# NVlabs/L4P

Hardware: AMD Instinct MI355X
Metric: frames/sec (all heads), 16x224x224 clip; encoder MFMA-roofline % (higher is better)
Workload: dtype bf16; 1 GPU; configs[2]: single MI355X, all heads (depth+flow+track2d/3d+motion-seg+pose), bf16, batch=4 clips, 64 track queries per clip; parallelism=dp1 (clips sharded, no collective in the step)

## Files before the change

### include/l4p_hip.h

```cpp
#ifndef L4P_HIP_H
#define L4P_HIP_H

#include <stddef.h>
#include <stdint.h>

#ifdef __cplusplus
extern "C" {
#endif

#define L4P_BF16 0
#define L4P_F32 1
#define L4P_F16 2

#define L4P_OK 0
#define L4P_E_INVALID (-1)
#define L4P_E_HIP (-2)
#define L4P_E_MISSING (-3)

typedef void* l4p_stream;
typedef struct l4p_engine l4p_engine;

const char* l4p_last_error(void);
int l4p_abi_version(void);

// ... 36 lines not shown
    float* out_f32;
    void* out_T;
    long long ldc;
    int epi;
    void* vt;
    int S, H, Dp;
    int kt, kh, kw, Cout;
    int a_gr, a_gs, a_go;
    int c_gr, c_gs, c_go;
    void* out_relu_T;
    void* k_tiled;
    int splitk;
    float* partial;
    const float* hyper;
    int hyper_rows;
    float q_scale;
    int tuning;
    int w_gr;
    long long w_gs;
    int b_gs;
    long long o_gs;
    int ups_hi, ups_wi;
    int kw_cols, kw_len;
} l4p_gemm_desc;

int l4p_gemm(l4p_stream stream, int dtype, const l4p_gemm_desc* d);
#define L4P_GEMM_GROUP_MAX 4
int l4p_gemm_group(l4p_stream stream, int dtype, const l4p_gemm_desc* d, int n);
int l4p_conv3d_k3(l4p_stream stream, int dtype, const l4p_gemm_desc* d);
int l4p_conv3d_subpixel(l4p_stream stream, int dtype, const l4p_gemm_desc* d);

int l4p_layernorm(l4p_stream stream, int dtype, const float* x, const float* gamma, const float* beta, float eps,
                  void* out_T, float* out_f32, int M, int C);

#define L4P_ATTN_PRESCALED 0.0f
int l4p_attention(l4p_stream stream, int dtype, const void* q, const void* kt, const void* vt, void* out, int B, int S,
                  int H, int Dh, float scale);

int l4p_patch_gather(l4p_stream stream, int dtype, const float* rgb, void* out, int B, int Cin, int T, int H, int W,
                     int pt, int ph, int pw, int Kp);

int l4p_cast(l4p_stream stream, int dtype, const float* x, void* y, long long n);

int l4p_upsample_trilinear(l4p_stream stream, int dtype, const void* x, void* y, int B, int Ti, int Hi, int Wi, int To,
                           int Ho, int Wo, int C, int align_corners);

// ... 225 lines not shown
```

### l4p_amd/_lib.py

```python
from __future__ import annotations

import ctypes as C
import os
from typing import Optional

L4P_BF16 = 0
L4P_F32 = 1
L4P_F16 = 2

ABI_VERSION = 17

EPI_DENSE, EPI_QKV, EPI_CONVT, EPI_MASKDOT = 0, 1, 2, 3
ACT_NONE, ACT_GELU, ACT_RELU = 0, 1, 2

_HERE = os.path.dirname(os.path.abspath(__file__))
LIB_PATH = os.environ.get("L4P_HIP_LIB") or os.path.join(_HERE, "lib", "libl4p_hip.so")


class GemmDesc(C.Structure):

    _fields_ = [
        ("A", C.c_void_p), ("lda", C.c_longlong),
        ("W", C.c_void_p), ("ldw", C.c_longlong),
        ("M", C.c_int), ("N", C.c_int), ("K", C.c_int),
        ("Ti", C.c_int), ("Hi", C.c_int), ("Wi", C.c_int), ("Cin", C.c_int),
        ("To", C.c_int), ("Ho", C.c_int), ("Wo", C.c_int),
        ("st", C.c_int), ("sh", C.c_int), ("sw", C.c_int), ("relu_in", C.c_int),
        ("bias", C.c_void_p), ("act", C.c_int),
        ("res1", C.c_void_p), ("res2", C.c_void_p), ("res_f32", C.c_int),
        ("ldr", C.c_longlong), ("res_mod", C.c_int),
        ("out_f32", C.c_void_p), ("out_T", C.c_void_p), ("ldc", C.c_longlong),
        ("epi", C.c_int),
        ("vt", C.c_void_p), ("S", C.c_int), ("H", C.c_int), ("Dp", C.c_int),
        ("kt", C.c_int), ("kh", C.c_int), ("kw", C.c_int), ("Cout", C.c_int),
        ("a_gr", C.c_int), ("a_gs", C.c_int), ("a_go", C.c_int),
        ("c_gr", C.c_int), ("c_gs", C.c_int), ("c_go", C.c_int),
        ("out_relu_T", C.c_void_p),
        ("k_tiled", C.c_void_p),
        ("splitk", C.c_int), ("partial", C.c_void_p),
        ("hyper", C.c_void_p), ("hyper_rows", C.c_int),
        ("q_scale", C.c_float), ("tuning", C.c_int),
        ("w_gr", C.c_int), ("w_gs", C.c_longlong), ("b_gs", C.c_int), ("o_gs", C.c_longlong),
        ("ups_hi", C.c_int), ("ups_wi", C.c_int),
        ("kw_cols", C.c_int), ("kw_len", C.c_int),
    ]


class EncoderCfg(C.Structure):

    _fields_ = [
        ("dim", C.c_int), ("depth", C.c_int), ("heads", C.c_int), ("head_dim", C.c_int), ("mlp_hidden", C.c_int),
        ("in_chans", C.c_int), ("frames", C.c_int), ("img_h", C.c_int), ("img_w", C.c_int),
        ("pt", C.c_int), ("ph", C.c_int), ("pw", C.c_int),
        ("patch_kp", C.c_int), ("ln_eps", C.c_float),
    ]


class DptCfg(C.Structure):

    _fields_ = [
        ("dim", C.c_int), ("nt", C.c_int), ("nh", C.c_int), ("nw", C.c_int),
        ("layer_dims", C.c_int * 4),
        ("feature_dim", C.c_int), ("last_dim", C.c_int), ("out_ch", C.c_int),
        ("actpost", (C.c_int * 3) * 4), ("fusion", (C.c_int * 3) * 4),
        ("out_t", C.c_int), ("out_h", C.c_int), ("out_w", C.c_int),
        ("post_exp", C.c_int),
    ]
# ... 166 lines not shown
```

### l4p_amd/csrc/api.hip

```cpp
#include <stdarg.h>
#include <stdio.h>
#include <string.h>

#include <string>
#include <unordered_map>
#include <vector>

#include <stdlib.h>

#include "engine.hpp"

static thread_local char g_err[512] = "";

void l4p_set_error(const char* fmt, ...) {
    va_list ap;
    va_start(ap, fmt);
    vsnprintf(g_err, sizeof(g_err), fmt, ap);
    va_end(ap);
}

int launch_layernorm_res(int dtype, const float* x, int x_mod, const void* delta_T, const float* gamma, const float* beta, float eps,
                         void* out_T, float* out_f32, int M, int C, const float* add, int add_mod, void* out_T2, const float* x_shared,
                         int x_period, int x_split, hipStream_t stream, float* out_sum = nullptr, const float* part = nullptr,
                         int nsplit = 0, const float* pbias = nullptr, float* out_stats = nullptr);

extern "C" {

const char* l4p_last_error(void) { return g_err; }
int l4p_abi_version(void) { return 17; }

int l4p_stream_create_cu_mask(int first_cu, int n_cus, l4p_stream* out) {
    if (!out || first_cu < 0 || n_cus < 1 || first_cu + n_cus > 1024) {
        l4p_set_error("l4p_stream_create_cu_mask: bad CU range [%d, %d)", first_cu, first_cu + n_cus);
        return L4P_E_INVALID;
    }
    uint32_t mask[32] = {0};
    for (int c = first_cu; c < first_cu + n_cus; ++c) mask[c >> 5] |= 1u << (c & 31);
    hipStream_t s = nullptr;
    HIP_TRY(hipExtStreamCreateWithCUMask(&s, (uint32_t)((first_cu + n_cus + 31) / 32), mask));
    *out = (l4p_stream)s;
    return 0;
}
int l4p_stream_destroy(l4p_stream s) {
    HIP_TRY(hipStreamDestroy((hipStream_t)s));
    return 0;
}

int l4p_gemm(l4p_stream stream, int dtype, const l4p_gemm_desc* d) {
    if (!d) {
        l4p_set_error("l4p_gemm: null descriptor");
        return L4P_E_INVALID;
    }
// ... 396 lines not shown
```

### l4p_amd/csrc/api_dpt.hip

```cpp
#include <string.h>

#include <string>

#include "engine.hpp"

namespace {

struct Bump {
    char* base;
    size_t off, cap;
    bool dry;
    void* take(size_t bytes) {
        const size_t a = (off + 255) & ~(size_t)255;
        off = a + bytes;
        return dry ? (void*)1 : (off <= cap ? base + a : nullptr);
    }
};

struct Vol {
    void* p;
    int t, h, w, c;
    long long vox(int B) const { return (long long)B * t * h * w; }
};

// ... 97 lines not shown
        if (rc || dry) return o;
        GemmParams p;
        memset(&p, 0, sizeof(p));
        p.A = x.p;
        p.W = W(wk);
        p.ldw = (long long)(k[0] == 1 ? 3 : 2) * (k[1] == 1 ? 3 : 2) * (k[2] == 1 ? 3 : 2) * x.c;
        p.M = (int)x.vox(B);
        p.N = k[0] * k[1] * k[2] * cout;
        p.K = (int)p.ldw;
        p.Ti = x.t;
        p.Hi = x.h;
        p.Wi = x.w;
        p.Cin = x.c;
        p.bias = (const float*)W(bk);
        p.out_T = o.p;
        p.out_relu_T = relu_copy ? relu_copy->p : nullptr;
        p.kt = k[0];
        p.kh = k[1];
        p.kw = k[2];
        p.Cout = cout;
        if (!rc) rc = launch_gemm(dt, 2, p, st);
        return o;
    }
    Vol conv3(const Vol& x_in, const char* wk, const char* bk, int cout, const int s[3], int act, const void* r1, const void* r2,
              Vol* relu_copy, int ups_h = 0, int ups_w = 0) {
        Vol x = x_in;
        if (ups_h > 0) x.h = ups_h, x.w = ups_w;
        Vol o = vol((x.t - 1) / s[0] + 1, (x.h - 1) / s[1] + 1, (x.w - 1) / s[2] + 1, cout);
        if (relu_copy) *relu_copy = vol(o.t, o.h, o.w, cout);
        const long long M = o.vox(B);
        const int sk = ups_h > 0 ? 1 : splitk_for(M, cout, 27 * x.c, es);
        float* partial = sk > 1 ? (float*)alloc((size_t)sk * M * cout * 4) : nullptr;
        if (rc || dry) return o;
        GemmParams p;
        memset(&p, 0, sizeof(p));
        p.A = x.p;
        p.W = W(wk);
        p.ldw = 27 * x.c;
        p.M = (int)M;
        p.N = cout;
        p.K = 27 * x.c;
        p.Ti = x.t;
        p.Hi = x.h;
        p.Wi = x.w;
        p.Cin = x.c;
        p.To = o.t;
        p.Ho = o.h;
        p.Wo = o.w;
        p.st = s[0];
        p.sh = s[1];
        p.sw = s[2];
        p.bias = bk ? (const float*)W(bk) : nullptr;
        p.act = act;
        if (r1) {
            p.res1 = r1;
            p.res2 = r2;
            p.res_f32 = 0;
            p.ldr = cout;
        }
        p.out_T = o.p;
        p.ldc = cout;
        p.out_relu_T = relu_copy ? relu_copy->p : nullptr;
        p.splitk = sk;
        p.partial = partial;
        if (ups_h > 0) p.ups_hi = x_in.h, p.ups_wi = x_in.w;
        if (!rc) rc = launch_gemm(dt, 1, p, st);
        return o;
    }
    Vol resize(const Vol& x, int t, int h, int w) {
        if (t == x.t && h == x.h && w == x.w) return x;
        Vol o = vol(t, h, w, x.c);
        if (rc || dry) return o;
        rc = launch_upsample(dt, x.p, o.p, B, x.t, x.h, x.w, t, h, w, x.c, 1, st);
        return o;
    }
};

int run(Ctx& c, const l4p_dpt_cfg* cfg, const void* const* hooks, float* out) {
    static const int one[3] = {1, 1, 1};
    const int F = cfg->feature_dim;
    Vol lay[4], layr[4];
    for (int i = 0; i < 4; ++i) {
        Vol tok{(void*)hooks[i], cfg->nt, cfg->nh, cfg->nw, cfg->dim};
        char wk[32], bk[32];
        snprintf(wk, sizeof(wk), "act%d.0.w", i);
        snprintf(bk, sizeof(bk), "act%d.0.b", i);
        Vol a = c.dense(tok, wk, bk, cfg->layer_dims[i]);
        const int* sf = cfg->actpost[i];
// ... 39 lines not shown
                return L4P_E_INVALID;
            }
            o = rcu(r, 1, lay[i], layr[i], p4.p, &orl);
        }
        Vol o2 = rcu(r, 2, o, orl, nullptr, nullptr);
        char wk[32], bk[32];
        snprintf(wk, sizeof(wk), "ref%d.out.w", r);
        snprintf(bk, sizeof(bk), "ref%d.out.b", r);
        Vol oc = c.dense(o2, wk, bk, F);
        const int* fs = cfg->fusion[i];
        path = c.resize(oc, oc.t * fs[0], oc.h * fs[1], oc.w * fs[2]);
        if (c.rc) return c.rc;
    }
    Vol h1 = c.conv3(path, "head1.w", "head1.b", F / 2, one, ACT_NONE, nullptr, nullptr, nullptr);
    Vol h2;
    const bool fuse = is16(c.dt) && knob(KNOB_CONV_UPS) && cfg->out_t == h1.t && (cfg->out_h != h1.h || cfg->out_w != h1.w) &&
                      cfg->last_dim == 128 && h1.c % 32 == 0 && cfg->out_t % 2 == 0 && cfg->out_h % 16 == 0 && cfg->out_w % 16 == 0 &&
                      (long long)c.B * cfg->out_t * cfg->out_h * cfg->out_w / 512 >= 192 &&
                      (long long)c.B * cfg->out_t * cfg->out_h * cfg->out_w * h1.c * 2 < (1ll << 32);
    if (fuse && !c.dry) {
        h2 = c.conv3(h1, "head2.w", "head2.b", cfg->last_dim, one, ACT_RELU, nullptr, nullptr, nullptr, cfg->out_h, cfg->out_w);
    } else {
        Vol h1u = c.resize(h1, cfg->out_t, cfg->out_h, cfg->out_w);
        h2 = c.conv3(h1u, "head2.w", "head2.b", cfg->last_dim, one, ACT_RELU, nullptr, nullptr, nullptr);
    }
    if (c.rc || c.dry) return c.rc;
    return launch_head_out(c.dt, h2.p, (const float*)c.W("out.w"), (const float*)c.W("out.b"), out,
                           (long long)h2.t * h2.h * h2.w, c.B, cfg->last_dim, cfg->out_ch, cfg->post_exp, c.st);
}

}

extern "C" {

size_t l4p_dpt_workspace_bytes(const l4p_engine* e, const l4p_dpt_cfg* cfg, int B) {
    if (!e || !cfg || B <= 0) return 0;
    Ctx c;
    c.e = e;
    c.st = nullptr;
    c.dt = e->dtype;
    c.es = esize_of(e->dtype);
    c.B = B;
    c.ws = Bump{nullptr, 0, 0, true};
    c.dry = true;
    const void* hooks[4] = {(void*)1, (void*)1, (void*)1, (void*)1};
    run(c, cfg, hooks, nullptr);
// ... 21 lines not shown
```

### l4p_amd/csrc/conv3_halo.hpp

```cpp
#pragma once
#include "gemm.hpp"

template <int WR, int WC>
struct ConvHaloCfg {
    static constexpr int BM = WR * 128, BN = WC * 64, CK = 32;
    static constexpr int TT = 2, TW = 16, TH = BM / (TT * TW);
    static constexpr int HH = TH + 2, HW = TW + 2, PR = HH * HW, NPL = TT + 2;
    static constexpr int PRP = (PR + 15) / 16 * 16;
    static constexpr int HALO_BYTES = NPL * PRP * 64;
    static constexpr int WSLOT = BN * 64, NSLOT = 4;
    static constexpr int LDS_BYTES = HALO_BYTES + NSLOT * WSLOT;
    static constexpr int W_PASS = BN * 4 / 512;
    static constexpr int H_PASS = (PRP * 4 + 511) / 512;
};

template <typename T, int WR, int WC, bool UPS = false>
__global__ __launch_bounds__(512) void conv3_halo_kernel(const GemmParams p) {
    static_assert(WR * WC == 8 && (WC == 2 || WC == 4), "8 waves");
    typedef ConvHaloCfg<WR, WC> Cfg;
    constexpr int BM = Cfg::BM, BN = Cfg::BN, TM = 8, TN = 4;
    constexpr int TT = Cfg::TT, TH = Cfg::TH, TW = Cfg::TW, HH = Cfg::HH, HW = Cfg::HW, PR = Cfg::PR, PRP = Cfg::PRP;
    constexpr int WSLOT = Cfg::WSLOT, W_PASS = Cfg::W_PASS, H_PASS = Cfg::H_PASS;
    static_assert(2 * H_PASS <= 9, "planes 2 / 3 are refilled before tap 9");
    typedef const __attribute__((address_space(1))) void* gptr_t;
    typedef __attribute__((address_space(3))) void* lptr_t;

    extern __shared__ __attribute__((aligned(16))) char smem[];
    char* const wring = smem + Cfg::HALO_BYTES;

    const int tid = threadIdx.x, lane = tid & 63;
    const int wave = __builtin_amdgcn_readfirstlane(tid >> 6);
    const int wr = wave / WC, wc = wave % WC, grp = wave >> 2;
    const int li = lane & 15, kg = lane >> 4;

    const int nbw = p.Wo / TW, nbh = p.Ho / TH, nbt = p.To / TT;
    const int ntiles = (p.M / BM);
    int tile;
    {
        const int bid = (int)blockIdx.x, xcd = bid & 7, idx = bid >> 3, q = ntiles >> 3, r = ntiles & 7;
        tile = (xcd < r ? xcd * (q + 1) : r * (q + 1) + (xcd - r) * q) + idx;
    }
    int rem = tile;
#ifdef CONV_HALO_ORDER_WTH
    const int bw = rem % nbw;
    rem /= nbw;
    const int bt = rem % nbt;
    rem /= nbt;
#else
    const int bt = rem % nbt;
    rem /= nbt;
    const int bw = rem % nbw;
    rem /= nbw;
#endif
// ... 246 lines not shown
                    tap = 0;
                    ++cs;
                    toff = (-PRP - HW) * 64;
                }
            }
        }
        koff3 += tap_bytes;
        if (++tap3 == 27) {
            tap3 = 0;
            koff3 += 64 - 27 * tap_bytes;
        }
    }
    if (grp == 0) __builtin_amdgcn_s_barrier();
    asm volatile("s_waitcnt vmcnt(0)" ::: "memory");

    const long long origin = (((long long)bb * p.To + t0) * p.Ho + h0) * p.Wo + w0;
    const int m_tile = tile * BM;
    const long long hw_out = (long long)p.Ho * p.Wo;
    const int Wo = p.Wo;
    auto rowmap = [=](int m) -> long long {
        const int r = m - m_tile, f = r >> 4;
        return origin + (long long)(f / TH) * hw_out + (f % TH) * Wo + (r & 15);
    };
    gemm_epilogue_dense_cases<T, TM, TN>(p, acc, m_tile + wr * 128, wc * 64, li, kg, rowmap);
}
```

### l4p_amd/csrc/gemm.hip

```cpp
#include "gemm.hpp"
int launch_gemm_bf16(int mode, const GemmParams& p, hipStream_t stream);
int launch_gemm_f16(int mode, const GemmParams& p, hipStream_t stream);
int launch_gemm_f32(int mode, const GemmParams& p, hipStream_t stream);

static int launch_subpixel_checked(int dtype, const GemmParams& d, hipStream_t stream) {
    const int es = esize_of(dtype);
    GemmParams p = d;
    const long long ksub = (long long)p.kt * p.kh * p.kw;
    if (p.kt < 1 || p.kh < 1 || p.kw < 1 || ksub < 2 || ksub > 64 || p.Ti < 1 || p.Hi < 1 || p.Wi < 1 || p.Cin < 1 || p.Cout < 1 || p.M <= 0) {
        l4p_set_error("conv3d_subpixel: needs strides kt, kh, kw >= 1 (at least one axis up-scaled, at most 64 sub-positions), a grid and channels");
        return L4P_E_INVALID;
    }
    const int cells = (p.kt == 1 ? 3 : 2) * (p.kh == 1 ? 3 : 2) * (p.kw == 1 ? 3 : 2);
    if (p.Cin % (128 / es) || p.Cout % 128 || p.N != ksub * p.Cout || p.M % (p.Ti * p.Hi * p.Wi) || p.ldw < (long long)cells * p.Cin || (p.ldw * es) % 16) {
        l4p_set_error("conv3d_subpixel: Cin %% %d, Cout %% 128, N == kt*kh*kw*Cout, M == B*Ti*Hi*Wi, ldw >= %d*Cin", 128 / es, cells);
        return L4P_E_INVALID;
    }
    if (p.Ti * p.kt < 2 || p.Hi * p.kh < 2 || p.Wi * p.kw < 2) {
        l4p_set_error("conv3d_subpixel: every up-scaled axis must be at least 2 long (three border classes per axis)");
        return L4P_E_INVALID;
    }
    if (!p.out_T || p.out_f32 || p.res1 || p.res2 || p.act != L4P_ACT_NONE || p.relu_in || p.splitk > 1 || p.a_gr > 0 || p.c_gr > 0 || p.w_gr > 0 ||
        p.kw_cols > 0 || p.ups_hi > 0 || (long long)p.M * ksub * p.Cout >= (1ll << 40)) {
        l4p_set_error("conv3d_subpixel: out_T (+ out_relu_T) only: no residual, activation, split-K, row maps or grouped weights");
        return L4P_E_INVALID;
    }
    p.To = p.Ti, p.Ho = p.Hi, p.Wo = p.Wi;
    p.st = p.sh = p.sw = 1;
    p.K = (int)p.ldw;
    p.epi = L4P_EPI_CONVT;
    return dtype == L4P_BF16 ? launch_gemm_bf16(2, p, stream) : dtype == L4P_F16 ? launch_gemm_f16(2, p, stream) : launch_gemm_f32(2, p, stream);
}

int launch_gemm(int dtype, int mode, const GemmParams& p, hipStream_t stream) {
    if (!dtype_ok(dtype)) { l4p_set_error("gemm: unknown dtype %d", dtype); return L4P_E_INVALID; }
    if (mode == 2) return launch_subpixel_checked(dtype, p, stream);
    const int es = esize_of(dtype);
    if (p.M <= 0 || p.N <= 0 || p.K <= 0) { l4p_set_error("gemm: empty problem M=%d N=%d K=%d", p.M, p.N, p.K); return L4P_E_INVALID; }
    if (p.N % 8) { l4p_set_error("gemm: N=%d must be a multiple of 8", p.N); return L4P_E_INVALID; }
    if ((p.K * es) % 16 || (p.ldw * es) % 16) { l4p_set_error("gemm: K/ldw not 16-byte aligned"); return L4P_E_INVALID; }
    if (mode == 0 && (p.lda * es) % 16) { l4p_set_error("gemm: lda not 16-byte aligned"); return L4P_E_INVALID; }
    if (mode == 1 && (p.Cin % (128 / es) || p.K != 27 * p.Cin)) { l4p_set_error("conv3d: Cin=%d must be a multiple of %d and K=27*Cin", p.Cin, 128 / es); return L4P_E_INVALID; }
    if (p.ups_hi > 0 && (mode != 1 || !is16(dtype) || p.ups_wi <= 0 || p.To != p.Ti)) {
        l4p_set_error("conv3d: the fused up-sampling loader (ups_hi / ups_wi) exists for l4p_conv3d_k3 on the 16-bit engines, time axis not resized");
        return L4P_E_INVALID;
    }
    if (p.splitk > 1) {
        const int bk = 128 / es, nk = (p.K + bk - 1) / bk;
        if (p.epi != L4P_EPI_DENSE || !p.partial || p.splitk > nk || p.c_gr > 0) {
            l4p_set_error("gemm: split-K needs the dense epilogue, a partial buffer and splitk <= %d k-tiles", nk);
            return L4P_E_INVALID;
        }
    }
    return dtype == L4P_BF16 ? launch_gemm_bf16(mode, p, stream) : dtype == L4P_F16 ? launch_gemm_f16(mode, p, stream) : launch_gemm_f32(mode, p, stream);
}

int launch_gemm_group_bf16(const GemmParams* p, int n, hipStream_t stream);
int launch_gemm_group_f16(const GemmParams* p, int n, hipStream_t stream);
int launch_gemm_group(int dtype, const GemmParams* p, int n, hipStream_t stream) {
    if (!p || n < 1 || n > L4P_GEMM_GROUP_MAX) {
        l4p_set_error("gemm_group: 1 <= n <= %d descriptors", L4P_GEMM_GROUP_MAX);
        return L4P_E_INVALID;
    }
    if (is16(dtype)) {
        for (int i = 0; i < n; ++i) {
            if (p[i].M <= 0 || p[i].N <= 0 || p[i].K <= 0 || p[i].N % 8 || (p[i].K * 2) % 16 || (p[i].ldw * 2) % 16 || (p[i].lda * 2) % 16 ||
                p[i].splitk > 1)
                goto one_by_one;
        }
        return dtype == L4P_F16 ? launch_gemm_group_f16(p, n, stream) : launch_gemm_group_bf16(p, n, stream);
    }
one_by_one:
    for (int i = 0; i < n; ++i) {
        const int rc = launch_gemm(dtype, 0, p[i], stream);
        if (rc) return rc;
    }
    return 0;
}
```

### l4p_amd/csrc/gemm_launch.inc

```
#include <cstdlib>
#include <cstring>

#include "gemm.hpp"
#include "prof.hpp"

template <typename T>
__global__ void splitk_finish_kernel(const GemmParams p) {
    const long long total = (long long)p.M * (p.N / 8);
    for (long long i = blockIdx.x * (long long)blockDim.x + threadIdx.x; i < total; i += (long long)gridDim.x * blockDim.x) {
        const int m = (int)(i / (p.N / 8)), n = (int)(i % (p.N / 8)) * 8;
        float v[8] = {0.f, 0.f, 0.f, 0.f, 0.f, 0.f, 0.f, 0.f};
        for (int s = 0; s < p.splitk; ++s) {
            const float* pp = p.partial + ((long long)s * p.M + m) * p.N + n;
            const f32x4 a = *(const f32x4*)pp, b = *(const f32x4*)(pp + 4);
#pragma unroll
            for (int q = 0; q < 4; ++q) {
                v[q] += a[q];
                v[4 + q] += b[q];
            }
        }
        if (p.bias) {
#pragma unroll
            for (int q = 0; q < 8; ++q) v[q] += p.bias[n + q];
        }
// ... 149 lines not shown
    if (p.tuning & 1) return false;
    if (p.epi == L4P_EPI_QKV) return !p.res1 && p.act == L4P_ACT_NONE && p.c_gr == 0;
    if (p.epi == L4P_EPI_CONVT) return !p.res1 && p.act == L4P_ACT_NONE && p.out_T && !p.out_f32 && !p.out_relu_T;
    return dense_epilogue_is_lean(p);
}
template <int WR, int WC>
static bool conv_halo_fits(const GemmParams& p) {
    typedef ConvHaloCfg<WR, WC> Cfg;
    if (p.ups_hi > 0 && !(WR == 4 && WC == 2 && p.ups_wi > 0 && (long long)p.ups_hi * p.ups_wi * p.Cin * 2 < (1ll << 31))) return false;
    return p.N == Cfg::BN && p.st == 1 && p.sh == 1 && p.sw == 1 && p.Cin % 32 == 0 && p.To % Cfg::TT == 0 && p.Ho % Cfg::TH == 0 &&
           p.Wo % Cfg::TW == 0 && p.To == p.Ti && p.Ho == p.Hi && p.Wo == p.Wi && p.M / Cfg::BM >= 192 && p.ldc == p.N &&
           (!p.res1 || p.ldr == p.N) && (long long)p.M * p.Cin * 2 < (1ll << 32) && !p.relu_in && p.splitk <= 1 && dense_epilogue_is_lean(p);
}
template <int WR, int WC, bool UPS = false>
static int launch_halo(const GemmParams& p, hipStream_t stream) {
    typedef ConvHaloCfg<WR, WC> Cfg;
    auto kern = conv3_halo_kernel<GEMM_T, WR, WC, UPS>;
    static lds_attr_state attr_done;
    HIP_TRY(lds_attr_once(attr_done, kern, Cfg::LDS_BYTES));
    ProfScope prof(PROF_CONV3D, stream, "M%d N%d K%d epi%d act%d halo%s t%dx%d", p.M, p.N, p.K, p.epi, p.act, UPS ? " ups" : "", Cfg::BM, Cfg::BN);
    hipLaunchKernelGGL(kern, dim3(p.M / Cfg::BM), dim3(512), Cfg::LDS_BYTES, stream, p);
    HIP_TRY(hipGetLastError());
    return 0;
}
#endif

static int GEMM_FN_impl(int mode, const GemmParams& p, hipStream_t stream);
int GEMM_FN(int mode, const GemmParams& p_in, hipStream_t stream);
#ifdef GEMM_HAS_8P
static bool gemm_is_skinny(const GemmParams& p) {
    const int max_m = knob(KNOB_SKINNY_MAX_M);
    return knob(KNOB_GEMM_SKINNY) && p.M >= 1 && p.M <= max_m && p.K >= 64 && p.K % 64 == 0 && p.lda % 8 == 0 && p.ldw % 8 == 0 && p.N % 8 == 0 &&
           p.w_gr == 0 && p.kw_cols == 0 && p.splitk <= 1 && !p.relu_in && p.epi == L4P_EPI_DENSE && !(p.tuning & 4) &&
           (long long)((p.M + 15) / 16) * ((p.N + 31) / 32) <= 512;
}
static bool gemm_is_skinny_grouped(const GemmParams& p) {
    return knob(KNOB_GEMM_SKINNY) && p.w_gr > 0 && p.w_gr % 16 == 0 && p.M >= 1 && p.M <= 2048 && p.K >= 64 && p.K % 64 == 0 && p.lda % 8 == 0 &&
           p.ldw % 8 == 0 && p.N % 8 == 0 && p.a_gr == 0 && p.splitk <= 1 && !p.relu_in && p.epi == L4P_EPI_DENSE && !(p.tuning & 4) &&
           (long long)((p.M + 15) / 16) * ((p.N + 31) / 32) <= 512;
}
static int launch_skinny(const GemmParams& p, hipStream_t stream) {
    const int grid = ((p.M + 15) / 16) * ((p.N + 31) / 32);
    ProfScope prof(PROF_GEMM_SMALL, stream, "M%d N%d K%d epi%d act%d%s skinny", p.M, p.N, p.K, p.epi, p.act, p.w_gr > 0 ? " wgrp" : "");
    if (p.w_gr > 0)
        hipLaunchKernelGGL((gemm_skinny_kernel<GEMM_T, true>), dim3(grid), dim3(64), 0, stream, p);
    else
// ... 125 lines not shown
    if (p.w_gr > 0) {
        if (mode != 0 || p.splitk > 1 || p.relu_in || p.w_gr % 128 || p.K % 8) {
            l4p_set_error("l4p_gemm: row-grouped weights need a dense GEMM without split-K, w_gr a multiple of 128");
            return L4P_E_INVALID;
        }
#ifdef GEMM_HAS_8P
        if (gemm_is_skinny_grouped(p)) return launch_skinny(p, stream);
        if (knob(KNOB_TRACK_DEEP) && p.N <= 64 && (long long)((p.M + 127) / 128) <= 256 && p.K >= 6 * 64) {
            if ((p.M + 127) / 128 <= 128 && p.w_gr % 64 == 0) return launch_cfg<64, 64, 0, true, 4, 2, 2, true>(p, stream);
            return launch_cfg<128, 64, 0, true, 4, 2, 2, true>(p, stream);
        }
#endif
        return p.N <= 64 ? launch_cfg<128, 64, 0, true, 2, 2, 2, true>(p, stream) : launch_cfg<128, 128, 0, true, 2, 2, 2, true>(p, stream);
    }
#ifdef GEMM_HAS_8P
    if (mode == 0 && gemm_is_skinny(p)) return launch_skinny(p, stream);
#endif
    const long long t128 = (long long)((p.M + 127) / 128) * ((p.N + 127) / 128);
    const bool big = (t128 >= 400 && !(t128 > 512 && t128 < 640)) || (p.splitk > 1 && p.N >= 256);
    const int variant = knob(KNOB_GEMM_VARIANT);
#ifdef GEMM_HAS_8P
    {
        const int halo = knob(KNOB_CONV_HALO);
        if (mode == 1 && p.ups_hi > 0) {
#ifdef L4P_PROBE_KERNELS
            if (conv_halo_fits<4, 2>(p)) return launch_halo<4, 2, true>(p, stream);
#else
            l4p_set_error("conv3d: the fused up-sampling loader (l4p_gemm_desc.ups_hi) is a measured-and-not-adopted form: build with PROBES=1");
            return L4P_E_INVALID;
#endif
            l4p_set_error("conv3d: the fused up-sampling loader takes N == 128, stride 1, Cin %% 32 == 0, whole 2 x 16 x 16 output blocks");
            return L4P_E_INVALID;
        }
        if (mode == 1 && halo && variant != 1) {
            if (conv_halo_fits<2, 4>(p)) return launch_halo<2, 4>(p, stream);
            if (conv_halo_fits<4, 2>(p)) return launch_halo<4, 2>(p, stream);
        }
    }
    if (p.splitk > 1 && mode == 0 && !p.relu_in && p.K % 8 == 0 && variant != 1 && p.N > 128) {
        const long long w8 = (long long)((p.M + 255) / 256) * ((p.N + 255) / 256) * p.splitk;
        const int t192sk = knob(KNOB_GEMM_T192);
        const long long w192 = (long long)((p.M + 255) / 256) * ((p.N + 191) / 192) * p.splitk;
        if (t192sk && w192 > w8 && w192 <= 256 && w8 >= 144 && p.K / p.splitk >= 512) return launch_8p<0, 4, 2, true, 4, 6>(p, stream);
        if (w8 >= 144 && w8 <= 256 && p.K / p.splitk >= 512) return launch_8p<0, 2, 4, true>(p, stream);
    }
    if (p.splitk <= 1 && !p.relu_in && p.K % 8 == 0 && variant != 1 && p.N > 128) {
// ... 39 lines not shown
```

### l4p_amd/csrc/prof.hip

```cpp
#include "prof.hpp"

#include <algorithm>
#include <atomic>
#include <cstdlib>
#include <cstring>
#include <map>
#include <mutex>
#include <string>
#include <vector>

#include "common.hpp"

bool g_prof_on = false;

namespace {
struct KnobDef {
    const char* name;
    const char* env;
    int dflt;
};
const KnobDef kKnobs[KNOB_NUM] = {{"conv_halo", "L4P_CONV_HALO", 1}, {"gemm_4w", "L4P_GEMM_4W", 0},
                                   {"maskdot_mfma", "L4P_MASKDOT_MFMA", 1},
                                   {"conv_ups", "L4P_CONV_UPS", 0},
                                   {"ln_tracks", "L4P_LN_TRACKS", 1},
// ... 5 lines not shown
                                   {"track_fold_l0", "L4P_TRACK_FOLD_L0", 1},
                                   {"track_fold_t2i", "L4P_TRACK_FOLD_T2I", 1},
                                   {"track_fold_t2i_v", "L4P_TRACK_FOLD_T2I_V", 1},
                                   {"track_kwin", "L4P_TRACK_KWIN", 1},
                                   {"track_ln_chain", "L4P_TRACK_LN_CHAIN", 1},
                                   {"track_fold_i2t", "L4P_TRACK_FOLD_I2T", 1},
                                   {"track_fold_pair", "L4P_TRACK_FOLD_PAIR", 0},
                                   {"track_delta_kernel", "L4P_TRACK_DELTA_KERNEL", 1},
                                   {"gemm_persist", "L4P_GEMM_PERSIST", 1},
                                   {"skinny_max_m", "L4P_SKINNY_MAX_M", 128},
                                   {"gemm_deep", "L4P_GEMM_DEEP", 1},
                                   {"gemm_group", "L4P_GEMM_GROUP", 1},
                                   {"epi_generic", "L4P_EPI_GENERIC", 0},
                                   {"gemm_variant", "L4P_GEMM_VARIANT", 0},
                                   {"gemm_t192", "L4P_GEMM_T192", 1},
                                   {"attn_persist", "L4P_ATTN_PERSIST", 1},
                                   {"attn_variant", "L4P_ATTN_VARIANT", 0},
                                   {"ups_ipt", "L4P_UPS_IPT", 2},
                                   {"ups_nt", "L4P_UPS_NT", 1},
                                   {"fc2_splitk8", "L4P_FC2_SPLITK8", -1},
                                   {"enc_defer_res", "L4P_ENC_DEFER_RES", 1},
                                   {"enc_sk_in_ln", "L4P_ENC_SK_IN_LN", 1},
                                   {"dpt_fold_rn", "L4P_DPT_FOLD_RN", 1},
                                   {"probe_kernels", "", 0}};
std::atomic<int> g_knob[KNOB_NUM];
std::once_flag g_knob_once;
#ifdef L4P_PROBE_KERNELS
constexpr bool kProbeKernels = true;
#else
constexpr bool kProbeKernels = false;
#endif
bool probe_only(int i) { return i == KNOB_GEMM_4W || i == KNOB_CONV_UPS; }
void knobs_init() {
    for (int i = 0; i < KNOB_NUM; ++i) {
        const char* e = kKnobs[i].env[0] ? getenv(kKnobs[i].env) : nullptr;
        int v = e ? atoi(e) : kKnobs[i].dflt;
        if (i == KNOB_PROBE_KERNELS) v = kProbeKernels ? 1 : 0;
        if (probe_only(i) && !kProbeKernels) v = 0;
        g_knob[i].store(v, std::memory_order_relaxed);
    }
}
}
int knob(int id) {
    std::call_once(g_knob_once, knobs_init);
    return g_knob[id].load(std::memory_order_relaxed);
}
// ... 120 lines not shown
```

### l4p_amd/csrc/prof.hpp

```cpp
#pragma once
#include <hip/hip_runtime.h>

#include <cstdarg>
#include <cstdio>

enum ProfClass {
    PROF_GEMM = 0,
    PROF_CONV3D,
    PROF_ATTENTION,
    PROF_LAYERNORM,
    PROF_ELEMENTWISE,
    PROF_TRACK,
    PROF_PREP,
    PROF_GEMM_SMALL,
    PROF_NUM
};

enum Knob {
    KNOB_CONV_HALO = 0, KNOB_GEMM_4W, KNOB_MASKDOT_MFMA, KNOB_CONV_UPS, KNOB_LN_TRACKS, KNOB_LN_ROWS16, KNOB_ATTN64, KNOB_GEMM_SKINNY,
    KNOB_READOUT_WIDE, KNOB_TRACK_DEEP,
    KNOB_TRACK_FOLD_L0, KNOB_TRACK_FOLD_T2I, KNOB_TRACK_FOLD_T2I_V, KNOB_TRACK_KWIN, KNOB_TRACK_LN_CHAIN, KNOB_TRACK_FOLD_I2T,
    KNOB_TRACK_FOLD_PAIR, KNOB_TRACK_DELTA_KERNEL,
    KNOB_GEMM_PERSIST, KNOB_SKINNY_MAX_M, KNOB_GEMM_DEEP, KNOB_GEMM_GROUP, KNOB_EPI_GENERIC, KNOB_GEMM_VARIANT, KNOB_GEMM_T192,
    KNOB_ATTN_PERSIST, KNOB_ATTN_VARIANT, KNOB_UPS_IPT, KNOB_UPS_NT, KNOB_FC2_SPLITK8, KNOB_ENC_DEFER_RES, KNOB_ENC_SK_IN_LN,
    KNOB_DPT_FOLD_RN,
    KNOB_PROBE_KERNELS, KNOB_NUM
};
int knob(int id);

void prof_begin(int cls, hipStream_t stream, const char* tag = nullptr);
void prof_end(int cls, hipStream_t stream);
extern bool g_prof_on;

struct ProfScope {
    int cls;
    hipStream_t s;
    ProfScope(int c, hipStream_t st) : cls(c), s(st) {
        if (g_prof_on) prof_begin(cls, s);
    }
    ProfScope(int c, hipStream_t st, const char* fmt, ...) __attribute__((format(printf, 4, 5))) : cls(c), s(st) {
        if (!g_prof_on) return;
        char tag[64];
        va_list ap;
        va_start(ap, fmt);
        vsnprintf(tag, sizeof tag, fmt, ap);
        va_end(ap);
        prof_begin(cls, s, tag);
    }
// ... 5 lines not shown
```

### l4p_amd/ops.py

```python
from __future__ import annotations

import ctypes as C
from typing import Optional, Tuple

import torch

from . import _lib
from ._lib import ACT_GELU, ACT_NONE, ACT_RELU, EPI_CONVT, EPI_DENSE, EPI_QKV, L4P_BF16, L4P_F16, L4P_F32, GemmDesc

DP = 96


def torch_dtype(dtype: int) -> torch.dtype:
    return {L4P_BF16: torch.bfloat16, L4P_F16: torch.float16, L4P_F32: torch.float32}[dtype]


def code_of(t: torch.dtype) -> int:
    if t == torch.bfloat16:
        return L4P_BF16
    if t == torch.float16:
        return L4P_F16
    if t == torch.float32:
        return L4P_F32
    raise ValueError(f"unsupported engine dtype {t}")
# ... 122 lines not shown
    assert dp == DP and tuple(q.shape) == (B * S, H * DP) and kt.numel() == q.numel()
    out = torch.empty((B * S, H * head_dim), dtype=q.dtype, device=q.device)
    scale = head_dim ** -0.5 if scale is None else scale
    lib = _lib.load()
    _lib.check(lib.l4p_attention(_stream(), code_of(q.dtype), _p(q), _p(kt), _p(vt), _p(out), B, S, H, head_dim, scale),
               "l4p_attention")
    return out


def patch_gather(rgb: torch.Tensor, patch: Tuple[int, int, int], kp: int, dtype: int) -> torch.Tensor:
    B, Cin, T, H, W = rgb.shape
    pt, ph, pw = patch
    tokens = (T // pt) * (H // ph) * (W // pw)
    out = torch.empty((B * tokens, kp), dtype=torch_dtype(dtype), device=rgb.device)
    lib = _lib.load()
    _lib.check(lib.l4p_patch_gather(_stream(), dtype, _p(rgb), _p(out), B, Cin, T, H, W, pt, ph, pw, kp),
               "l4p_patch_gather")
    return out


def conv3d_k3(x: torch.Tensor, w: torch.Tensor, cout: int, *, stride: Tuple[int, int, int] = (1, 1, 1),
              bias: Optional[torch.Tensor] = None, relu_in: bool = False, act: int = ACT_NONE,
              res1: Optional[torch.Tensor] = None, res2: Optional[torch.Tensor] = None, relu_copy: bool = False,
              ups_to: Optional[Tuple[int, int]] = None):
    dtype = code_of(x.dtype)
    B, Ti, Hi, Wi, Cin = x.shape
    lo = None
    if ups_to is not None:
        lo, (Hi, Wi) = (Hi, Wi), ups_to
    st, sh, sw = stride
    To, Ho, Wo = (Ti - 1) // st + 1, (Hi - 1) // sh + 1, (Wi - 1) // sw + 1
    out = torch.empty((B, To, Ho, Wo, cout), dtype=x.dtype, device=x.device)
    d = GemmDesc()
    d.A, d.W, d.ldw = _p(x), _p(w), 27 * Cin
    d.M, d.N, d.K = B * To * Ho * Wo, cout, 27 * Cin
    d.Ti, d.Hi, d.Wi, d.Cin, d.To, d.Ho, d.Wo = Ti, Hi, Wi, Cin, To, Ho, Wo
    d.st, d.sh, d.sw, d.relu_in = st, sh, sw, 1 if relu_in else 0
    d.bias, d.act = _p(bias), act
    if res1 is not None:
        d.res1, d.res2, d.res_f32, d.ldr = _p(res1), _p(res2), 0, cout
    d.out_T, d.ldc = _p(out), cout
    if lo is not None:
        d.ups_hi, d.ups_wi = lo
    out_relu = torch.empty_like(out) if relu_copy else None
    d.out_relu_T = _p(out_relu)
    sk = splitk_for(d.M, cout, 27 * Cin, x.element_size()) if lo is None else 1
    if sk > 1:
        partial = torch.empty((sk, d.M, cout), dtype=torch.float32, device=x.device)
        d.splitk, d.partial = sk, _p(partial)
    lib = _lib.load()
    _lib.check(lib.l4p_conv3d_k3(_stream(), dtype, C.byref(d)), "l4p_conv3d_k3")
    return (out, out_relu) if relu_copy else out


def conv3d_subpixel(x: torch.Tensor, w: torch.Tensor, cout: int, k: Tuple[int, int, int], bias_cls: Optional[torch.Tensor] = None,
                    relu_copy: bool = False):
    dtype = code_of(x.dtype)
    B, Ti, Hi, Wi, Cin = x.shape
    kt, kh, kw = k
    out = torch.empty((B, Ti * kt, Hi * kh, Wi * kw, cout), dtype=x.dtype, device=x.device)
    assert w.dtype == x.dtype and w.shape[0] >= kt * kh * kw * cout
    d = GemmDesc()
    d.A, d.W, d.ldw = _p(x), _p(w), w.shape[1]
    d.M, d.N, d.K = B * Ti * Hi * Wi, kt * kh * kw * cout, w.shape[1]
    d.Ti, d.Hi, d.Wi, d.Cin = Ti, Hi, Wi, Cin
    d.bias = _p(bias_cls)
    d.out_T = _p(out)
    out_relu = torch.empty_like(out) if relu_copy else None
    d.out_relu_T = _p(out_relu)
    d.kt, d.kh, d.kw, d.Cout = kt, kh, kw, cout
    lib = _lib.load()
    _lib.check(lib.l4p_conv3d_subpixel(_stream(), dtype, C.byref(d)), "l4p_conv3d_subpixel")
    return (out, out_relu) if relu_copy else out

# ... 42 lines not shown
```

Measured before the change: 994.7 frames/s.

## Fuse DPT head output 1x1 projection into the halo conv3 epilogue

Adds a head-out epilogue variant of the halo 3x3x3 conv kernel. After bias+ReLU, the 128-channel tile is staged in LDS with a swizzle, and each thread applies the small 1x1 output projection (up to 8 channels, optional exp) and writes the fp32 result straight to the head output. The DPT head path uses it when the shape constraints and the new knob allow, which skips materialising the 128-channel activation and the separate output conv launch. In exchange the kernel needs extra LDS, an extra block barrier, and per-thread scalar dot products in the epilogue.

Result: no change. 996.5 frames/s, median of 4 (+0.2%).

```diff
diff --git a/include/l4p_hip.h b/include/l4p_hip.h
--- a/include/l4p_hip.h
+++ b/include/l4p_hip.h
@@ -82,6 +82,12 @@
     long long o_gs;
     int ups_hi, ups_wi;
     int kw_cols, kw_len;
+    const float* ho_w;
+    const float* ho_b;
+    float* ho_out;
+    int ho_cout;
+    int ho_exp;
+    long long ho_vox;
 } l4p_gemm_desc;
 
 int l4p_gemm(l4p_stream stream, int dtype, const l4p_gemm_desc* d);
diff --git a/l4p_amd/_lib.py b/l4p_amd/_lib.py
--- a/l4p_amd/_lib.py
+++ b/l4p_amd/_lib.py
@@ -8,7 +8,7 @@
 L4P_F32 = 1
 L4P_F16 = 2
 
-ABI_VERSION = 17
+ABI_VERSION = 18
 
 EPI_DENSE, EPI_QKV, EPI_CONVT, EPI_MASKDOT = 0, 1, 2, 3
 ACT_NONE, ACT_GELU, ACT_RELU = 0, 1, 2
@@ -43,6 +43,8 @@
         ("w_gr", C.c_int), ("w_gs", C.c_longlong), ("b_gs", C.c_int), ("o_gs", C.c_longlong),
         ("ups_hi", C.c_int), ("ups_wi", C.c_int),
         ("kw_cols", C.c_int), ("kw_len", C.c_int),
+        ("ho_w", C.c_void_p), ("ho_b", C.c_void_p), ("ho_out", C.c_void_p),
+        ("ho_cout", C.c_int), ("ho_exp", C.c_int), ("ho_vox", C.c_longlong),
     ]
 
 
diff --git a/l4p_amd/csrc/api.hip b/l4p_amd/csrc/api.hip
--- a/l4p_amd/csrc/api.hip
+++ b/l4p_amd/csrc/api.hip
@@ -27,7 +27,7 @@
 extern "C" {
 
 const char* l4p_last_error(void) { return g_err; }
-int l4p_abi_version(void) { return 17; }
+int l4p_abi_version(void) { return 18; }
 
 int l4p_stream_create_cu_mask(int first_cu, int n_cus, l4p_stream* out) {
     if (!out || first_cu < 0 || n_cus < 1 || first_cu + n_cus > 1024) {
diff --git a/l4p_amd/csrc/api_dpt.hip b/l4p_amd/csrc/api_dpt.hip
--- a/l4p_amd/csrc/api_dpt.hip
+++ b/l4p_amd/csrc/api_dpt.hip
@@ -143,11 +143,16 @@
         if (!rc) rc = launch_gemm(dt, 2, p, st);
         return o;
     }
+    struct HeadOut {
+        const float *w, *b;
+        float* out;
+        int cout, post_exp;
+    };
     Vol conv3(const Vol& x_in, const char* wk, const char* bk, int cout, const int s[3], int act, const void* r1, const void* r2,
-              Vol* relu_copy, int ups_h = 0, int ups_w = 0) {
+              Vol* relu_copy, int ups_h = 0, int ups_w = 0, const HeadOut* ho = nullptr) {
         Vol x = x_in;
         if (ups_h > 0) x.h = ups_h, x.w = ups_w;
-        Vol o = vol((x.t - 1) / s[0] + 1, (x.h - 1) / s[1] + 1, (x.w - 1) / s[2] + 1, cout);
+        Vol o = ho ? Vol{nullptr, x.t, x.h, x.w, cout} : vol((x.t - 1) / s[0] + 1, (x.h - 1) / s[1] + 1, (x.w - 1) / s[2] + 1, cout);
         if (relu_copy) *relu_copy = vol(o.t, o.h, o.w, cout);
         const long long M = o.vox(B);
         const int sk = ups_h > 0 ? 1 : splitk_for(M, cout, 27 * x.c, es);
@@ -185,6 +190,11 @@
         p.splitk = sk;
         p.partial = partial;
         if (ups_h > 0) p.ups_hi = x_in.h, p.ups_wi = x_in.w;
+        if (ho) {
+            p.ho_w = ho->w, p.ho_b = ho->b, p.ho_out = ho->out;
+            p.ho_cout = ho->cout, p.ho_exp = ho->post_exp;
+            p.ho_vox = (long long)o.t * o.h * o.w;
+        }
         if (!rc) rc = launch_gemm(dt, 1, p, st);
         return o;
     }
@@ -270,6 +280,17 @@
         h2 = c.conv3(h1, "head2.w", "head2.b", cfg->last_dim, one, ACT_RELU, nullptr, nullptr, nullptr, cfg->out_h, cfg->out_w);
     } else {
         Vol h1u = c.resize(h1, cfg->out_t, cfg->out_h, cfg->out_w);
+        const long long vox = (long long)cfg->out_t * cfg->out_h * cfg->out_w;
+        const bool ho_fits = is16(c.dt) && knob(KNOB_DPT_HEAD_OUT) && knob(KNOB_CONV_HALO) && knob(KNOB_GEMM_VARIANT) != 1 &&
+                             !knob(KNOB_EPI_GENERIC) && cfg->last_dim == 128 && cfg->out_ch >= 1 && cfg->out_ch <= 8 && h1u.c % 32 == 0 &&
+                             cfg->out_t % 2 == 0 && cfg->out_h % 16 == 0 && cfg->out_w % 16 == 0 && c.B * vox / 512 >= 192 &&
+                             c.B * vox * h1u.c * 2 < (1ll << 32) && c.B * vox < (1ll << 31);
+        if (ho_fits && !c.dry) {
+            const Ctx::HeadOut ho{(const float*)c.W("out.w"), (const float*)c.W("out.b"), out, cfg->out_ch, cfg->post_exp};
+            if (c.rc) return c.rc;
+            c.conv3(h1u, "head2.w", "head2.b", cfg->last_dim, one, ACT_RELU, nullptr, nullptr, nullptr, 0, 0, &ho);
+            return c.rc;
+        }
         h2 = c.conv3(h1u, "head2.w", "head2.b", cfg->last_dim, one, ACT_RELU, nullptr, nullptr, nullptr);
     }
     if (c.rc || c.dry) return c.rc;
diff --git a/l4p_amd/csrc/conv3_halo.hpp b/l4p_amd/csrc/conv3_halo.hpp
--- a/l4p_amd/csrc/conv3_halo.hpp
+++ b/l4p_amd/csrc/conv3_halo.hpp
@@ -14,9 +14,19 @@
     static constexpr int H_PASS = (PRP * 4 + 511) / 512;
 };
 
-template <typename T, int WR, int WC, bool UPS = false>
-__global__ __launch_bounds__(512) void conv3_halo_kernel(const GemmParams p) {
+template <int WR, int WC>
+struct ConvHaloHoCfg {
+    typedef ConvHaloCfg<WR, WC> Cfg;
+    static constexpr int ROWB = Cfg::BN * 2;
+    static constexpr int TILE_BYTES = Cfg::BM * ROWB;
+    static constexpr int WS_FLOATS = 8 * Cfg::BN + 8;
+    static constexpr int LDS_BYTES = (TILE_BYTES > Cfg::LDS_BYTES ? TILE_BYTES : Cfg::LDS_BYTES) + WS_FLOATS * 4;
+};
+
+template <typename T, int WR, int WC, bool UPS, bool HO>
+__device__ __forceinline__ void conv3_halo_body(const GemmParams& p) {
     static_assert(WR * WC == 8 && (WC == 2 || WC == 4), "8 waves");
+    static_assert(!HO || (WR == 4 && WC == 2 && !UPS && sizeof(T) == 2), "head-out epilogue: the 512 x 128 form of the 16-bit engines");
     typedef ConvHaloCfg<WR, WC> Cfg;
     constexpr int BM = Cfg::BM, BN = Cfg::BN, TM = 8, TN = 4;
     constexpr int TT = Cfg::TT, TH = Cfg::TH, TW = Cfg::TW, HH = Cfg::HH, HW = Cfg::HW, PR = Cfg::PR, PRP = Cfg::PRP;
@@ -29,6 +39,12 @@
     char* const wring = smem + Cfg::HALO_BYTES;
 
     const int tid = threadIdx.x, lane = tid & 63;
+    if constexpr (HO) {
+        typedef ConvHaloHoCfg<WR, WC> Ho;
+        float* const ws = (float*)(smem + Ho::LDS_BYTES - Ho::WS_FLOATS * 4);
+        for (int i = tid; i < p.ho_cout * Cfg::BN; i += 512) ws[i] = p.ho_w[i];
+        if (tid < p.ho_cout) ws[8 * Cfg::BN + tid] = p.ho_b[tid];
+    }
     const int wave = __builtin_amdgcn_readfirstlane(tid >> 6);
     const int wr = wave / WC, wc = wave % WC, grp = wave >> 2;
     const int li = lane & 15, kg = lane >> 4;
@@ -321,5 +337,76 @@
         const int r = m - m_tile, f = r >> 4;
         return origin + (long long)(f / TH) * hw_out + (f % TH) * Wo + (r & 15);
     };
-    gemm_epilogue_dense_cases<T, TM, TN>(p, acc, m_tile + wr * 128, wc * 64, li, kg, rowmap);
+    if constexpr (HO) {
+        typedef ConvHaloHoCfg<WR, WC> Ho;
+        constexpr int ROWB = Ho::ROWB, C = BN;
+        static_assert(ROWB / 16 == 16, "the swizzle below assumes 16 chunks per row");
+        const float* const ws = (const float*)(smem + Ho::LDS_BYTES - Ho::WS_FLOATS * 4);
+        __syncthreads();
+        const int nb = wc * 64 + 16 * kg;
+        float bv[16];
+#pragma unroll
+        for (int g = 0; g < 4; ++g) {
+            const f32x4 z = {0.f, 0.f, 0.f, 0.f};
+            const f32x4 b4 = p.bias ? *(const f32x4*)(p.bias + nb + 4 * g) : z;
+#pragma unroll
+            for (int q = 0; q < 4; ++q) bv[4 * g + q] = b4[q];
+        }
+        epi_static_for<0, TM>([&](auto i_) {
+            constexpr int i = decltype(i_)::value;
+            const int r = wr * 128 + i * 16 + li;
+            const long long off = rowmap(m_tile + r) * p.ldc + nb;
+#pragma unroll
+            for (int g = 0; g < 2; ++g) {
+                vec8h<T> o;
+#pragma unroll
+                for (int q = 0; q < 8; ++q) {
+                    float x = acc[i][2 * g + q / 4][q % 4] + bv[8 * g + q];
+                    x = fmaxf(x, 0.f);
+                    o[q] = (T)x;
+                }
+                if (p.out_T) *(vec8h<T>*)((T*)p.out_T + off + 8 * g) = o;
+                *(vec8h<T>*)(smem + r * ROWB + ((((nb >> 3) + g) ^ (r & 15)) << 4)) = o;
+            }
+        });
+        __syncthreads();
+        const int Cout = p.ho_cout;
+        float a8[8];
+#pragma unroll
+        for (int o = 0; o < 8; ++o) a8[o] = 0.f;
+        const char* xr = smem + tid * ROWB;
+#pragma unroll 4
+        for (int c0 = 0; c0 < C; c0 += 8) {
+            const char* cp = xr + ((((c0 * (int)sizeof(T)) >> 4) ^ (tid & 15)) << 4);
+            float v[8];
+            const vec8h<T> t = *(const vec8h<T>*)cp;
+#pragma unroll
+            for (int k = 0; k < 8; ++k) v[k] = (float)t[k];
+#pragma unroll
+            for (int o = 0; o < 8; ++o)
+                if (o < Cout) {
+#pragma unroll
+                    for (int k = 0; k < 8; ++k) a8[o] += v[k] * ws[o * C + c0 + k];
+                }
+        }
+        const long long v = rowmap(m_tile + tid) - (long long)bb * p.ho_vox;
+#pragma unroll
+        for (int o = 0; o < 8; ++o)
+            if (o < Cout) {
+                float r = a8[o] + ws[8 * C + o];
+                if (p.ho_exp) r = expf(r);
+                p.ho_out[((long long)bb * Cout + o) * p.ho_vox + v] = r;
+            }
+    } else {
+        gemm_epilogue_dense_cases<T, TM, TN>(p, acc, m_tile + wr * 128, wc * 64, li, kg, rowmap);
+    }
 }
+
+template <typename T, int WR, int WC, bool UPS = false>
+__global__ __launch_bounds__(512) void conv3_halo_kernel(const GemmParams p) {
+    conv3_halo_body<T, WR, WC, UPS, false>(p);
+}
+template <typename T>
+__global__ __launch_bounds__(512) void conv3_halo_ho_kernel(const GemmParams p) {
+    conv3_halo_body<T, 4, 2, false, true>(p);
+}
diff --git a/l4p_amd/csrc/gemm.hip b/l4p_amd/csrc/gemm.hip
--- a/l4p_amd/csrc/gemm.hip
+++ b/l4p_amd/csrc/gemm.hip
@@ -21,7 +21,7 @@
         return L4P_E_INVALID;
     }
     if (!p.out_T || p.out_f32 || p.res1 || p.res2 || p.act != L4P_ACT_NONE || p.relu_in || p.splitk > 1 || p.a_gr > 0 || p.c_gr > 0 || p.w_gr > 0 ||
-        p.kw_cols > 0 || p.ups_hi > 0 || (long long)p.M * ksub * p.Cout >= (1ll << 40)) {
+        p.kw_cols > 0 || p.ups_hi > 0 || p.ho_cout != 0 || (long long)p.M * ksub * p.Cout >= (1ll << 40)) {
         l4p_set_error("conv3d_subpixel: out_T (+ out_relu_T) only: no residual, activation, split-K, row maps or grouped weights");
         return L4P_E_INVALID;
     }
@@ -45,6 +45,10 @@
         l4p_set_error("conv3d: the fused up-sampling loader (ups_hi / ups_wi) exists for l4p_conv3d_k3 on the 16-bit engines, time axis not resized");
         return L4P_E_INVALID;
     }
+    if (p.ho_cout != 0 && (mode != 1 || !is16(dtype) || p.ho_cout < 1 || p.ho_cout > 8)) {
+        l4p_set_error("conv3d: the head-out epilogue (ho_*) exists for l4p_conv3d_k3 on the 16-bit engines, 1 <= ho_cout <= 8 (ho_cout=%d)", p.ho_cout);
+        return L4P_E_INVALID;
+    }
     if (p.splitk > 1) {
         const int bk = 128 / es, nk = (p.K + bk - 1) / bk;
         if (p.epi != L4P_EPI_DENSE || !p.partial || p.splitk > nk || p.c_gr > 0) {
@@ -65,7 +69,7 @@
     if (is16(dtype)) {
         for (int i = 0; i < n; ++i) {
             if (p[i].M <= 0 || p[i].N <= 0 || p[i].K <= 0 || p[i].N % 8 || (p[i].K * 2) % 16 || (p[i].ldw * 2) % 16 || (p[i].lda * 2) % 16 ||
-                p[i].splitk > 1)
+                p[i].splitk > 1 || p[i].ho_cout != 0)
                 goto one_by_one;
         }
         return dtype == L4P_F16 ? launch_gemm_group_f16(p, n, stream) : launch_gemm_group_bf16(p, n, stream);
diff --git a/l4p_amd/csrc/gemm_launch.inc b/l4p_amd/csrc/gemm_launch.inc
--- a/l4p_amd/csrc/gemm_launch.inc
+++ b/l4p_amd/csrc/gemm_launch.inc
@@ -195,6 +195,25 @@
     hipLaunchKernelGGL(kern, dim3(p.M / Cfg::BM), dim3(512), Cfg::LDS_BYTES, stream, p);
     HIP_TRY(hipGetLastError());
     return 0;
+}
+static bool conv_halo_ho_fits(const GemmParams& p) {
+    if constexpr (sizeof(GEMM_T) != 2) return false;
+    return conv_halo_fits<4, 2>(p) && p.act == L4P_ACT_RELU && !p.res1 && !p.res2 && !p.out_relu_T && !p.out_f32 && p.splitk <= 1 && p.ups_hi == 0 &&
+           p.ho_cout >= 1 && p.ho_cout <= 8 && p.ho_w && p.ho_b && p.ho_out && p.ho_vox == (long long)p.To * p.Ho * p.Wo;
+}
+static int launch_halo_ho(const GemmParams& p, hipStream_t stream) {
+    if constexpr (sizeof(GEMM_T) == 2) {
+        typedef ConvHaloCfg<4, 2> Cfg;
+        typedef ConvHaloHoCfg<4, 2> Ho;
+        auto kern = conv3_halo_ho_kernel<GEMM_T>;
+        static lds_attr_state attr_done;
+        HIP_TRY(lds_attr_once(attr_done, kern, Ho::LDS_BYTES));
+        ProfScope prof(PROF_CONV3D, stream, "M%d N%d K%d epi%d act%d halo ho t%dx%d", p.M, p.N, p.K, p.epi, p.act, Cfg::BM, Cfg::BN);
+        hipLaunchKernelGGL(kern, dim3(p.M / Cfg::BM), dim3(512), Ho::LDS_BYTES, stream, p);
+        HIP_TRY(hipGetLastError());
+        return 0;
+    }
+    return L4P_E_INVALID;
 }
 #endif
 
@@ -366,6 +385,12 @@
 #ifdef GEMM_HAS_8P
     {
         const int halo = knob(KNOB_CONV_HALO);
+        if (p.ho_cout != 0) {
+            if (mode == 1 && conv_halo_ho_fits(p)) return launch_halo_ho(p, stream);
+            l4p_set_error("conv3d: the head-out epilogue (l4p_gemm_desc.ho_*) takes a 16-bit engine, N == 128, ReLU, no residual / second output / "
+                          "split-K / ups_hi, 1 <= ho_cout <= 8, ho_vox == To*Ho*Wo, stride 1, Cin %% 32 == 0, >= 192 whole 2 x 16 x 16 output blocks");
+            return L4P_E_INVALID;
+        }
         if (mode == 1 && p.ups_hi > 0) {
 #ifdef L4P_PROBE_KERNELS
             if (conv_halo_fits<4, 2>(p)) return launch_halo<4, 2, true>(p, stream);
diff --git a/l4p_amd/csrc/prof.hip b/l4p_amd/csrc/prof.hip
--- a/l4p_amd/csrc/prof.hip
+++ b/l4p_amd/csrc/prof.hip
@@ -51,6 +51,7 @@
                                    {"enc_defer_res", "L4P_ENC_DEFER_RES", 1},
                                    {"enc_sk_in_ln", "L4P_ENC_SK_IN_LN", 1},
                                    {"dpt_fold_rn", "L4P_DPT_FOLD_RN", 1},
+                                   {"dpt_head_out", "L4P_DPT_HEAD_OUT", 1},
                                    {"probe_kernels", "", 0}};
 std::atomic<int> g_knob[KNOB_NUM];
 std::once_flag g_knob_once;
diff --git a/l4p_amd/csrc/prof.hpp b/l4p_amd/csrc/prof.hpp
--- a/l4p_amd/csrc/prof.hpp
+++ b/l4p_amd/csrc/prof.hpp
@@ -23,7 +23,7 @@
     KNOB_TRACK_FOLD_PAIR, KNOB_TRACK_DELTA_KERNEL,
     KNOB_GEMM_PERSIST, KNOB_SKINNY_MAX_M, KNOB_GEMM_DEEP, KNOB_GEMM_GROUP, KNOB_EPI_GENERIC, KNOB_GEMM_VARIANT, KNOB_GEMM_T192,
     KNOB_ATTN_PERSIST, KNOB_ATTN_VARIANT, KNOB_UPS_IPT, KNOB_UPS_NT, KNOB_FC2_SPLITK8, KNOB_ENC_DEFER_RES, KNOB_ENC_SK_IN_LN,
-    KNOB_DPT_FOLD_RN,
+    KNOB_DPT_FOLD_RN, KNOB_DPT_HEAD_OUT,
     KNOB_PROBE_KERNELS, KNOB_NUM
 };
 int knob(int id);
diff --git a/l4p_amd/ops.py b/l4p_amd/ops.py
--- a/l4p_amd/ops.py
+++ b/l4p_amd/ops.py
@@ -168,7 +168,8 @@
 def conv3d_k3(x: torch.Tensor, w: torch.Tensor, cout: int, *, stride: Tuple[int, int, int] = (1, 1, 1),
               bias: Optional[torch.Tensor] = None, relu_in: bool = False, act: int = ACT_NONE,
               res1: Optional[torch.Tensor] = None, res2: Optional[torch.Tensor] = None, relu_copy: bool = False,
-              ups_to: Optional[Tuple[int, int]] = None):
+              ups_to: Optional[Tuple[int, int]] = None,
+              head_out: Optional[Tuple[torch.Tensor, torch.Tensor, bool]] = None, want_out: bool = True):
     dtype = code_of(x.dtype)
     B, Ti, Hi, Wi, Cin = x.shape
     lo = None
@@ -176,7 +177,7 @@
         lo, (Hi, Wi) = (Hi, Wi), ups_to
     st, sh, sw = stride
     To, Ho, Wo = (Ti - 1) // st + 1, (Hi - 1) // sh + 1, (Wi - 1) // sw + 1
-    out = torch.empty((B, To, Ho, Wo, cout), dtype=x.dtype, device=x.device)
+    out = torch.empty((B, To, Ho, Wo, cout), dtype=x.dtype, device=x.device) if (want_out or head_out is None) else None
     d = GemmDesc()
     d.A, d.W, d.ldw = _p(x), _p(w), 27 * Cin
     d.M, d.N, d.K = B * To * Ho * Wo, cout, 27 * Cin
@@ -190,12 +191,21 @@
         d.ups_hi, d.ups_wi = lo
     out_relu = torch.empty_like(out) if relu_copy else None
     d.out_relu_T = _p(out_relu)
+    y = None
+    if head_out is not None:
+        ho_w, ho_b, post_exp = head_out
+        assert ho_w.dtype == torch.float32 and ho_b.dtype == torch.float32 and ho_w.is_contiguous() and ho_w.shape[1] == cout
+        y = torch.empty((B, ho_w.shape[0], To, Ho, Wo), dtype=torch.float32, device=x.device)
+        d.ho_w, d.ho_b, d.ho_out = _p(ho_w), _p(ho_b), _p(y)
+        d.ho_cout, d.ho_exp, d.ho_vox = ho_w.shape[0], 1 if post_exp else 0, To * Ho * Wo
     sk = splitk_for(d.M, cout, 27 * Cin, x.element_size()) if lo is None else 1
     if sk > 1:
         partial = torch.empty((sk, d.M, cout), dtype=torch.float32, device=x.device)
         d.splitk, d.partial = sk, _p(partial)
     lib = _lib.load()
     _lib.check(lib.l4p_conv3d_k3(_stream(), dtype, C.byref(d)), "l4p_conv3d_k3")
+    if head_out is not None:
+        return out, y
     return (out, out_relu) if relu_copy else out
 
 
```
